# quadram-institute-bioscience/tatajuba

Measured on AMD Instinct MI355X. Metric: reads/s (whole node), 150 bp synthetic FASTQ, homopolymer scan + context histogram, higher is better.
Workload: dtype u8/u64

## Files before the change

tatajuba_amd/csrc/hopo_device.hip:

```cpp

#include <hip/hip_runtime.h>
#include <rccl/rccl.h>
#include <dlfcn.h>
#include <mutex>
#include <string>
#include <new>
#include <stdint.h>
#include <stdio.h>
#include <stdlib.h>
#include <string.h>
#include <stdarg.h>
#include <limits.h>
#include <float.h>
#include <algorithm>
#include <vector>

#include "../../include/tatajuba_amd.h"

typedef unsigned long long u64;
typedef unsigned int u32;


static thread_local char g_err[512] = "";

// ... 1736 lines not shown
#endif
#endif
        const u32 sh = u + u;
        const u32 clo = __builtin_amdgcn_alignbit (w1, w0, sh), chi = __builtin_amdgcn_alignbit (w2, w1, sh);
        const u32 l = clo & vkm;
        const u32 cb = (clo >> vk2) & 3u;
        const u32 r = (u32) ((((u64) chi << 32) | clo) >> (vk2 + len + len)) & vkm;
        u32 rcl = revcomp_v32 (l, M55, vrs), rcr = revcomp_v32 (r, M55, vrs);
        if ((ncand_all >= 0x40000000u)) {
          const u32 nb = bits32 (T.np, (int) u);
          if ((nb << ((v32 - need) & 31u)) != 0u && need <= 32u) {
            rcl = revcomp_v32 (l | (u32) spread_pairs (nb & ((1u << k) - 1u)), M55, vrs);
            rcr = revcomp_v32 (r | (u32) spread_pairs ((nb >> ((u32) k + len)) & ((1u << k) - 1u)), M55, vrs);
          }
        }
        const bool rev = cb >= 2u;
        const u32 c0 = rev ? rcr : l, c1 = rev ? rcl : r;
        const u32 fld24 = __builtin_amdgcn_perm (0u, 0x10140C08u, (cb << 24) | 0x000C0C0Cu);
        const u32 lo = c1 | (len << 24);
        const u32 hi = c0 | fld24;
        STAMP (6);
#if defined(FK_EXP_STOP) && FK_EXP_STOP == 3
        if (ok) asm volatile ("" :: "v"(lo), "v"(hi), "v"(at));
#else
#if defined(FK_EXP_LINEAR)
        {
          const u32 at = lds_collect (araw) + (u32) __builtin_amdgcn_mbcnt_hi ((u32) (okm >> 32), __builtin_amdgcn_mbcnt_lo ((u32) okm, 0u));
          typedef __attribute__((address_space(1))) u64 *gwords_t;
          gwords_t q = (gwords_t) ((u64) (size_t) BK.pool + (((u64) blockIdx.x * 200000u + (at % 200000u)) << 3));
          if (ok) *q = ((u64) hi << 32) | lo;
        }
#elif defined(FK_EXP_SCATTER)
        (void) lds_collect (araw);
        {
          u32 h = __builtin_amdgcn_udot4 (lo, vh0, 0u, false);
          h = __builtin_amdgcn_udot4 (hi & vm27, vh1, h, false);
          const u32 bin = ok ? ((h ^ (h >> 8)) & 255u) : 256u + (u32) lane;
          const u32 r = atomicAdd (&SL.hist[bin], 1u);
          const uint4 e = reinterpret_cast<const uint4 *> (SL.gbase)[bin & 255u];
          asm volatile ("" :: "v"(e.x), "v"(e.y), "v"(e.z), "v"(e.w));
          typedef __attribute__((address_space(1))) u64 *gwords_t;
          gwords_t q = (gwords_t) ((u64) (size_t) BK.pool + ((((u64) (bin & 255u) * 512u + (blockIdx.x & 511u)) * 512u + (r & 511u)) << 3));
          if (ok) *q = ((u64) hi << 32) | lo;
        }
#else
        const u32 at = lds_collect (araw) + (u32) __builtin_amdgcn_mbcnt_hi ((u32) (okm >> 32), __builtin_amdgcn_mbcnt_lo ((u32) okm, 0u));
        if constexpr (LOG) sink.store1ok (ok, at, lo, hi, (u32) lane);
        else sink.store1v (ok ? at : (u32) sink.S + (u32) lane, lo, hi, vh0, vh1, vm27);
#endif
#endif
        STAMP (7);
      }
    }
#if !(defined(FK_EXP_NOBAR) && (FK_EXP_NOBAR & 1))
    lds_barrier ();
#endif
    STAMP (8);
    if (nt >= grp_end) { gpar ^= 1u; grp_end = nt + FK_GROUP; }
    tile = nt;
    it++;
  }
  STAMP_FLUSH;
  flush_slow ();
  sink.finish ();
}

#define PL_BLOCK 512
#ifndef PL_WG_PER_CU
#define PL_WG_PER_CU 2
#endif
template <int W>
__global__ __launch_bounds__ (PL_BLOCK, PL_BLOCK * PL_WG_PER_CU / 256)
void partition_log_kernel (LogSpace LG, Buckets BK, DevCounters *ctr, int k)
{
  static_assert (W == 1 || W == 2, "the log holds one-word and two-word records");
  typedef StageLds<W, 2> Lds;
  __shared__ Lds L;
  constexpr u32 RB = TJ_LOGB / W;
  static_assert (Lds::S == (int) RB && Lds::WS == W, "one pass per log block");
  constexpr u32 RR = RB / PL_BLOCK;
  static_assert (RR % 4 == 0, "bins are kept four to a register");
  const u32 tid = threadIdx.x, lane = tid & 63u;
  const u32 wave = (u32) __builtin_amdgcn_readfirstlane ((int) (tid >> 6));
  if (tid < TJ_P) L.hist[tid] = 0;
  u32 cur_j = TJ_EMPTY, cur_chunk = TJ_NOCHUNK;
  lds_barrier ();
  const u32 n_blocks = min (*LG.next, LG.n_blocks);
#if TJ_STAMPS == 2
  Stamper stamper; stamper.begin ();
#endif
  u32 b = blockIdx.x;
  if (b >= n_blocks) return;
  u64 w[RR][W];
  u32 n = min (LG.count[b], RB), nn = 0;
  auto load_block = [&] (u32 blk, u32 cnt) {
    const u64 *__restrict__ src = LG.log + ((u64) blk << TJ_LOGB_SHIFT);
    const u32 w0 = tid & ~63u;
#pragma unroll
    for (u32 r = 0; r < RR; r++) {
#pragma unroll
      for (int j = 0; j < W; j++) w[r][j] = 0;
      if (w0 + r * PL_BLOCK < cnt) {
        if constexpr (W == 1) w[r][0] = (src + r * PL_BLOCK)[tid];
        else { const ulonglong2 v = reinterpret_cast<const ulonglong2 *> (src + 2u * r * PL_BLOCK)[tid]; w[r][0] = v.x; w[r][1] = v.y; }
      }
    }
  };
  auto bucket_of = [&] (const u64 *rec) -> u32 {
    if constexpr (W == 1) return bucket_of_rec1 ((u32) rec[0], (u32) (rec[0] >> 32));
    else { u64 c0, c1; u32 base, len10, flag; unpack_raw<W> (rec, k, c0, c1, base, len10, flag); return bucket_of_key (c0, c1, base, len10); }
  };
  load_block (b, n);
  while (true) {
    const u32 bn = b + gridDim.x;
    const bool more = bn < n_blocks;
    if (more) nn = min (LG.count[bn], RB);
    PLSTAMP (0);
    u32 tq = tid;
    asm volatile ("" : "+v"(tq));
    u32 pk[RR / 4];
#pragma unroll
    for (u32 r = 0; r < RR / 4; r++) pk[r] = 0;
    if (n) {
#pragma unroll
      for (u32 r = 0; r < RR; r++) {
        const u32 bin = bucket_of (w[r]);
        pk[r >> 2] |= bin << (8u * (r & 3u));
        if (tid + r * PL_BLOCK < n) atomicAdd (&L.hist[bin], 1u);
      }
      PLSTAMP (1);
      lds_barrier ();
      PLSTAMP (2);
      if (wave < TJ_P / 64) {
        const uint4 h4 = *reinterpret_cast<const uint4 *> (&L.hist[4 * lane]);
        const u32 tot = h4.x + h4.y + h4.z + h4.w;
        const u32 e0 = wave_inclusive_scan (tot) - tot;
        if ((lane >> 4) == wave) *reinterpret_cast<uint4 *> (&L.offs[4 * lane]) = make_uint4 (e0, e0 + h4.x, e0 + h4.x + h4.y, e0 + h4.x + h4.y + h4.z);
        const u32 cnt = L.hist[tid], off = L.offs[tid];
        u64 a1 = 0, a2 = 0;
        u32 thr = off + cnt;
        if (cnt) {
          const u32 p0 = atomicAdd (&BK.cursors[tid * TJ_CSTRIDE], cnt);
          const u32 ch = (u32) TJ_CH0 << BK.ch_shift;
          bucket_claim_ahead_range (BK, tid, p0, cnt, ctr);
          const u32 j0 = chunk_of_pos (BK, p0), j1 = chunk_of_pos (BK, p0 + cnt - 1);
          if (j0 != cur_j) { cur_j = j0; cur_chunk = bucket_chunk_id (BK, tid, j0, true, ctr); }
          if (cur_chunk != TJ_NOCHUNK) a1 = (u64) (size_t) (BK.pool + ((u64) cur_chunk * ch + (p0 - j0 * ch)) * W) - (8ull * W) * off;
          if (j1 != j0) {
            thr = off + ((j0 + 1u) * ch - p0);
            cur_j = j0 + 1u; cur_chunk = bucket_chunk_id (BK, tid, j0 + 1u, true, ctr);
            if (cur_chunk != TJ_NOCHUNK) a2 = (u64) (size_t) (BK.pool + ((u64) cur_chunk * ch) * W) - (8ull * W) * thr;
          }
        }
        reinterpret_cast<uint4 *> (L.gbase)[tid] = make_uint4 ((u32) a1, (u32) (a1 >> 32) | (thr << 16), (u32) a2, (u32) (a2 >> 32));
      }
      PLSTAMP (3);
      lds_barrier ();
      PLSTAMP (4);
      if (tid < TJ_P) L.hist[tid] = 0;
#pragma unroll
      for (u32 r = 0; r < RR; r++)
        if (tid + r * PL_BLOCK < n) {
          const u32 bin = (pk[r >> 2] >> (8u * (r & 3u))) & 255u;
          const u32 d = atomicAdd (&L.offs[bin], 1u);
#pragma unroll
          for (int j = 0; j < W; j++) L.rec[d * W + j] = w[r][j];
          L.bin[d] = (unsigned char) bin;
        }
      PLSTAMP (5);
      lds_barrier ();
      PLSTAMP (6);
      for (u32 r0 = 0; r0 < RR; r0 += 4) {
        if (r0 * PL_BLOCK >= n) break;
        u32 cb[4]; uint4 e[4]; u64 cw[4][W];
#pragma unroll
        for (u32 h = 0; h < 4; h++) cb[h] = L.bin[tq + (r0 + h) * PL_BLOCK];
#pragma unroll
        for (u32 h = 0; h < 4; h++) {
          e[h] = reinterpret_cast<const uint4 *> (L.gbase)[cb[h]];
#pragma unroll
          for (int j = 0; j < W; j++) cw[h][j] = L.rec[(tq + (r0 + h) * PL_BLOCK) * W + j];
        }
#pragma unroll
        for (u32 h = 0; h < 4; h++) {
          const u32 i = tq + (r0 + h) * PL_BLOCK;
          const u64 a = (i < (e[h].y >> 16)) ? (((u64) (e[h].y & 0xFFFFu) << 32) | e[h].x) : (((u64) e[h].w << 32) | e[h].z);
          if (i < n && a != 0ull) {
            typedef __attribute__((address_space(1))) u64 *gwords_t;
            gwords_t q = (gwords_t) (a + (u64) (8u * W * i));
#pragma unroll
            for (int j = 0; j < W; j++) q[j] = cw[h][j];
          }
        }
      }
      PLSTAMP (7);
      lds_barrier ();
      PLSTAMP (8);
    }
    if (!more) break;
    load_block (bn, nn);
    n = nn; b = bn;
  }
  PLSTAMP_FLUSH;
}

template <int W>
__global__ void nrun_fixup_bins_kernel (const uint8_t *__restrict__ seq, long n_bytes, int k, int mprime,
                                        Buckets BK, DevCounters *ctr, const FixEntry *fix, u32 fix_cap, int par)
{
  nrun_fixup_entries<W> (seq, n_bytes, k, mprime, BK, ctr, fix, fix_cap, par, blockIdx.x * (u64) blockDim.x + threadIdx.x, (u64) gridDim.x * blockDim.x);
}

template <int W>
__global__ void bin_elems_kernel (const u64 *__restrict__ elems5, long n, int k, Buckets BK, DevCounters *ctr)
{
  for (long i = blockIdx.x * (long) blockDim.x + threadIdx.x; i < n; i += (long) gridDim.x * blockDim.x) {
    const u64 m = elems5[5 * i + 2];
    bucket_insert_slow<W> (elems5[5 * i], elems5[5 * i + 1], (u32) (m & 3ull), (u32) ((m >> TJ_META_LEN_SHIFT) & 0x3FFull),
                           (u32) ((m >> TJ_META_FLAG_SHIFT) & 3ull), k, BK, ctr);
  }
}

template <int W>
__global__ void unpack_buckets_kernel (Buckets BK, int k, u64 *__restrict__ out, u64 cap, u64 *n_out)
{
  const u32 b = blockIdx.x;
  const u32 n = BK.cursors[b * TJ_CSTRIDE];
  for (u32 i = threadIdx.x; i < n; i += blockDim.x) {
    u64 c0, c1; u32 base, len10, flag;
    const u64 at = bucket_slot (BK, b, i, false, nullptr);
    if (at == ~0ull) continue;
    unpack_raw<W> (BK.pool + at * W, k, c0, c1, base, len10, flag);
    if (flag == 3u) continue;
    const u64 o = atomicAdd (n_out, 1ull);
    if (o < cap) { u64 *q = out + 3 * o; q[0] = c0; q[1] = c1; q[2] = make_meta (base, len10, flag); }
  }
}

__global__ void init_table_kernel (u32 *table, u32 maxj, u32 *pool_next)
{
  const u32 b = blockIdx.x * blockDim.x + threadIdx.x;
  if (b < TJ_P) table[(u64) b * maxj] = b;
  if (b == 0) *pool_next = TJ_P;
}

__global__ void clear_buckets_kernel (u32 *cursors, DevCounters *ctr, u32 *table, u32 maxj, int ch_shift, FinCounts *fin, u32 *bins, int nbins,
                                      DevCounters *snap_ctr, u32 *snap_cursors, FinPlan *plan, u32 *__restrict__ fine = nullptr, int fine_bits = 0)
{
  const u32 b = blockIdx.x;
  if (snap_ctr) {
    if (threadIdx.x == 0) {
      snap_cursors[b] = cursors[b * TJ_CSTRIDE];
      if (b == 0) {
        snap_cursors[TJ_P] = cursors[TJ_P * TJ_CSTRIDE];
        if (plan) { plan->n1_exact = (long) fin->n_kept; plan->ovf_exact = fin->overflow; }
      }
    }
    if (b == 0) for (u32 i = threadIdx.x; i < sizeof (DevCounters) / 4; i += blockDim.x) reinterpret_cast<u32 *> (snap_ctr)[i] = reinterpret_cast<const u32 *> (ctr)[i];
    __syncthreads ();
  }
  if (b == 0) for (u32 i = threadIdx.x; i < sizeof (DevCounters) / 4; i += blockDim.x) if (i != offsetof (DevCounters, n_undefined) / 4 && i != offsetof (DevCounters, n_undefined) / 4 + 1) reinterpret_cast<u32 *> (ctr)[i] = 0;
  if (table) {
    u32 used = maxj;
    if (ch_shift >= 0) used = min (maxj, ((cursors[b * TJ_CSTRIDE] / TJ_CH0) >> ch_shift) + 3u);
    for (u32 j = threadIdx.x; j < used; j += blockDim.x) table[(u64) b * maxj + j] = j ? TJ_EMPTY : b;
  }
  if (fine) {
    const int gid = (int) (b * blockDim.x + threadIdx.x), gsz = (int) (gridDim.x * blockDim.x);
    if (plan->ok) {
      const int shift = fine_bits - plan->nbits, run = 1 << shift, nb = plan->nbins;
      for (int i = gid; i < nb; i += gsz) {
        u32 sum = 0;
        if (shift >= 2) {
          uint4 *f4 = reinterpret_cast<uint4 *> (fine) + (size_t) i * (run >> 2);
          for (int j = 0; j < (run >> 2); j++) { const uint4 v = f4[j]; sum += v.x + v.y + v.z + v.w; }
          for (int j = 0; j < (run >> 2); j++) f4[j] = make_uint4 (0, 0, 0, 0);
        }
        else {
          for (int j = 0; j < run; j++) sum += fine[(i << shift) + j];
          for (int j = 0; j < run; j++) fine[(i << shift) + j] = 0;
        }
        bins[i] = sum;
      }
    }
    else for (int i = gid; i < (1 << fine_bits); i += gsz) fine[i] = 0;
  }
  else if (bins) for (int i = (int) (b * blockDim.x + threadIdx.x); i < nbins; i += (int) (gridDim.x * blockDim.x)) bins[i] = 0;
  __syncthreads ();
  if (threadIdx.x == 0) { cursors[b * TJ_CSTRIDE] = 0; if (b == 0) { cursors[TJ_P * TJ_CSTRIDE] = TJ_P; fin->n_kept = 0; fin->overflow = 0; fin->pad = 0; } }
}

__global__ void table_relayout_kernel (const u32 *__restrict__ old, u32 old_maxj, u32 *__restrict__ neu, u32 new_maxj)
{
  const u32 b = blockIdx.x;
  for (u32 j = threadIdx.x; j < old_maxj; j += blockDim.x) neu[(u64) b * new_maxj + j] = old[(u64) b * old_maxj + j];
}


#define AG_BLOCK    1024
#define AG_NCH      512

#define AG1_S        8192
#define AG1_CLOSE_AT 4864
#define AG1_R        4
#define AG1_MARK     (~0ull)

#define BS_MAXBITS   16
__host__ __device__ static inline int cov_table_bits (long n1) { int b = 10; while ((1l << b) < 4 * n1 && b < 31) b++; return b; }
__host__ __device__ static inline int cov_plan_bits (long n1, int k, int *direct)
{
  const int hb = cov_table_bits (n1), kb = 2 * k < 31 ? 2 * k : 31;
  *direct = kb <= hb ? 1 : 0;
  return kb <= hb ? kb : hb;
}
__host__ __device__ static inline int fine_bin_bits (int k) { return BS_MAXBITS < 1 + 4 * k ? BS_MAXBITS : 1 + 4 * k; }
__device__ __forceinline__ u32 bin_of_record (u64 c0, u64 c1, u64 meta, int k, int nbits);
__host__ __device__ static inline int bin_bits_for (long n1, int k)
{
  int nbits = 6;
  while (nbits < BS_MAXBITS && nbits < 1 + 4 * k && (48l << nbits) < n1) nbits++;
  return nbits < 1 + 4 * k ? nbits : 1 + 4 * k;
}
__device__ __forceinline__ void flag_kept_overflow (FinCounts *fin)
{
  u32 old = atomicOr (&fin->overflow, 1u);
  asm volatile ("" :: "v"(old));
}

__device__ __forceinline__ void plan_tail (FinCounts *fin, int k, long cap, FinPlan *plan)
{
  if (!plan) return;
  __syncthreads ();
  if (threadIdx.x == 0) {
    const u32 done = atomicAdd (&fin->pad, 1u);
    if (done == gridDim.x - 1u) {
      const long n1 = (long) __hip_atomic_load (&fin->n_kept, __ATOMIC_RELAXED, __HIP_MEMORY_SCOPE_AGENT);
      const u32 ovf = __hip_atomic_load (&fin->overflow, __ATOMIC_RELAXED, __HIP_MEMORY_SCOPE_AGENT);
      plan->n1 = n1; plan->kept_overflow = ovf;
      plan->nbits = bin_bits_for (n1, k); plan->nbins = 1 << plan->nbits;
      int direct;
      plan->log2t = cov_plan_bits (n1, k, &direct); plan->t = 1l << plan->log2t; plan->cov_direct = (u32) direct;
      plan->ok = (n1 > 0 && n1 <= cap && !ovf) ? 1 : 0;
      fin->pad = 0;
    }
  }
}

#ifndef AG_FROM_END
#define AG_FROM_END 1
#endif
__device__ __forceinline__ u32 batch_start (u32 t, u32 n, u32 batch)
{
#if AG_FROM_END
  const u32 nb = (n + batch - 1u) / batch;
  return t < nb ? (nb - 1u - t) * batch : n;
#else
  return t * batch;
#endif
}

struct Agg1Lds
{
  u64 key[AG1_S];
  u32 cnt[2 * AG1_S];
  u32 chunk[AG_NCH];
  u32 n_claimed, n_ovf, total;
  u32 next_batch;
  u32 wsum[AG_BLOCK / 64];
};

__global__ __launch_bounds__ (AG_BLOCK)
void aggregate1_kernel (Buckets BK, u64 *ovf, int k, int remove_biased, u64 *__restrict__ kept, u64 kept_cap, FinCounts *fin,
                        long plan_cap, FinPlan *plan, u32 *__restrict__ fine, int fine_bits)
{
  __shared__ Agg1Lds L;
  const int tid = threadIdx.x, lane = tid & 63, wave = tid >> 6;
  const u32 bkt = blockIdx.x;
  u32 n = BK.cursors[bkt * TJ_CSTRIDE];
  if (n) for (u32 j = (u32) tid; j <= chunk_of_pos (BK, n - 1u) && j < AG_NCH; j += AG_BLOCK) L.chunk[j] = bucket_chunk_id (BK, bkt, j, false, nullptr);
  auto chunk_id = [&] (u32 j) { return j < AG_NCH ? L.chunk[j] : bucket_chunk_id (BK, bkt, j, false, nullptr); };

  const u64 *src = BK.pool;
  u64 *dst = ovf;
  ASTAMP_DECL;
  while (n > 0) {
    ASTAMP (0);
    for (int i = tid; i < AG1_S; i += AG_BLOCK) { L.key[i] = 0; L.cnt[2 * i] = 0; L.cnt[2 * i + 1] = 0; }
    if (tid == 0) { L.n_claimed = 0; L.n_ovf = 0; L.next_batch = 0; }
    __syncthreads ();

    u64 wn[AG1_R];
    u32 vn = 0;
    auto fetch = [&] (u32 b0) {
      vn = 0;
#pragma unroll
      for (int r = 0; r < AG1_R; r++) wn[r] = 0;
      if (b0 >= n) return;
      const u32 ch = (u32) TJ_CH0 << BK.ch_shift;
      const u32 j0 = chunk_of_pos (BK, b0), bound = (j0 + 1u) * ch;
      if (b0 + 64u * AG1_R <= min (n, bound) && j0 < AG_NCH) {
        const u32 c0s = (u32) __builtin_amdgcn_readfirstlane ((int) L.chunk[j0]);
        if (c0s != TJ_NOCHUNK) {
          const u64 *q = src + ((u64) c0s * ch + (b0 - j0 * ch)) + (u32) lane;
#pragma unroll
          for (int r = 0; r < AG1_R; r++) wn[r] = q[64 * r];
          vn = (1u << AG1_R) - 1u;
          return;
        }
      }
      const u32 c0 = chunk_id (j0), c1 = (bound < n) ? chunk_id (j0 + 1u) : TJ_NOCHUNK;
      const u64 off0 = (u64) c0 * ch - (u64) j0 * ch, off1 = (u64) c1 * ch - (u64) bound;
#pragma unroll
      for (int r = 0; r < AG1_R; r++) {
        const u32 idx = b0 + (u32) r * 64u + (u32) lane;
        const bool hi = idx >= bound;
        if (idx < n && (hi ? c1 : c0) != TJ_NOCHUNK) { vn |= 1u << r; wn[r] = src[(hi ? off1 : off0) + idx]; }
      }
    };
    auto next_batch = [&] () {
      u32 b = 0;
      if (lane == 0) b = atomicAdd (&L.next_batch, 1u);
      return batch_start ((u32) __builtin_amdgcn_readfirstlane ((int) b), n, 64u * AG1_R);
    };
    u32 b_next = next_batch ();
    fetch (b_next);
    ASTAMP (1);
    while (b_next < n) {
      const u32 b0 = b_next;
      (void) b0;
      asm volatile ("s_waitcnt vmcnt(0)" : "+v"(wn[0]), "+v"(wn[1]), "+v"(wn[2]), "+v"(wn[3]) :: "memory");
      static_assert (AG1_R == 4, "asm operand list");
      ASTAMP (2);
      u64 w[AG1_R];
#pragma unroll
      for (int r = 0; r < AG1_R; r++) w[r] = wn[r];
      const u32 valid = vn;
      b_next = next_batch ();
      fetch (b_next);
      ASTAMP (3);
      ASTAMP (4);
#if defined(TJ_EXP_AGG) && TJ_EXP_AGG == 1
      { u64 acc = 0;
#pragma unroll
        for (int r = 0; r < AG1_R; r++) acc ^= w[r];
        if (acc == 0x123456789ull) atomicAdd (&L.n_ovf, 1u);
        continue; }
#endif
      {
        auto home = [] (u64 key) {
          u32 h = (u32) key ^ __builtin_amdgcn_alignbit ((u32) (key >> 32), (u32) (key >> 32), 17);
          h *= 0x9E3779B1u; h ^= h >> 15;
          return h & (AG1_S / 2 - 1);
        };
        u32 todo = 0;
        u32 hp[AG1_R];
        ulonglong2 hk[AG1_R];
#pragma unroll
        for (int r = 0; r < AG1_R; r++) {
          hp[r] = home (w[r] & R1_KEY_MASK);
          hk[r] = *reinterpret_cast<const ulonglong2 *> (&L.key[2 * hp[r]]);
        }
        asm volatile ("" : "+v"(hk[0].x), "+v"(hk[0].y), "+v"(hk[1].x), "+v"(hk[1].y), "+v"(hk[2].x), "+v"(hk[2].y), "+v"(hk[3].x), "+v"(hk[3].y));
#pragma unroll
        for (int r = 0; r < AG1_R; r++) {
          const u64 cur = w[r];
          if (((valid >> r) & 1u) && ((cur >> R1_FLAG_SHIFT) & 3ull) != 3ull) {
            const u64 key = cur & R1_KEY_MASK;
            const bool hx = hk[r].x == key, hy = hk[r].y == key;
            if (hx | hy) atomicAdd (&L.cnt[4 * hp[r] + (hx ? 0u : 2u) + ((u32) (cur >> (R1_FLAG_SHIFT + 1)) & 1u)], 1u);
            else todo |= 1u << r;
          }
        }
        u32 probes = 0;
        u32 r = todo ? (u32) __ffs ((int) todo) - 1u : 0u;
        u64 cur = (r == 0u) ? w[0] : (r == 1u) ? w[1] : (r == 2u) ? w[2] : w[3];
        u32 pair = home (cur & R1_KEY_MASK);
        while (todo) {
          bool adv = false, left = false;
          {
            const u64 key = cur & R1_KEY_MASK;
            const u32 strand = (u32) (cur >> (R1_FLAG_SHIFT + 1)) & 1u;
            const ulonglong2 kk = *reinterpret_cast<const ulonglong2 *> (&L.key[2 * pair]);
            if (kk.x == key || kk.y == key) { atomicAdd (&L.cnt[4 * pair + (kk.x == key ? 0u : 2u) + strand], 1u); adv = true; }
            else {
              const bool e0 = (kk.x == 0ull) | (kk.x == AG1_MARK), e1 = (kk.y == 0ull) | (kk.y == AG1_MARK);
              if (e0 | e1) {
                const u32 slot = 2 * pair + (e0 ? 0u : 1u);
                if ((e0 ? kk.x : kk.y) == AG1_MARK) { left = true; adv = true; }
                else {
                  const bool closed = __hip_atomic_load (&L.n_claimed, __ATOMIC_RELAXED, __HIP_MEMORY_SCOPE_WORKGROUP) > AG1_CLOSE_AT;
                  const u64 old = atomicCAS ((unsigned long long *) &L.key[slot], 0ull, closed ? AG1_MARK : (unsigned long long) key);
                  if (old == 0ull) {
                    if (closed) left = true;
                    else { atomicAdd (&L.n_claimed, 1u); atomicAdd (&L.cnt[2 * slot + strand], 1u); }
                    adv = true;
                  }
                }
              }
              else if (++probes >= AG1_S / 2) { left = true; adv = true; }
              else pair = (pair + 1u) & (AG1_S / 2 - 1);
            }
          }
          if (left) {
            const u32 o = atomicAdd (&L.n_ovf, 1u);
            const u32 j = chunk_of_pos (BK, o), oc = chunk_id (j);
            if (oc != TJ_NOCHUNK) dst[(((u64) oc * TJ_CH0) << BK.ch_shift) + (o - ((j * TJ_CH0) << BK.ch_shift))] = cur;
          }
          if (adv) {
            todo &= todo - 1u; probes = 0;
            if (todo) {
              r = (u32) __ffs ((int) todo) - 1u;
              cur = (r == 1u) ? w[1] : (r == 2u) ? w[2] : w[3];
              pair = home (cur & R1_KEY_MASK);
            }
          }
        }
      }
      ASTAMP (5);
    }
    __syncthreads ();
    ASTAMP (6);

    u32 mine = 0;
    u64 metas[AG1_S / AG_BLOCK];
#pragma unroll
    for (int r = 0; r < AG1_S / AG_BLOCK; r++) {
      const int slot = tid + r * AG_BLOCK;
      metas[r] = 0;
      if (L.key[slot] && L.key[slot] != AG1_MARK) {
        const u32 cf = L.cnt[2 * slot], cr = L.cnt[2 * slot + 1];
        const u64 flag = (cf ? 1ull : 0ull) | (cr ? 2ull : 0ull);
        const u64 cnt = ((u64) cf + (u64) cr) & 0xFFFFFull;
        const int scnt = (cnt & 0x80000ull) ? (int) cnt - 0x100000 : (int) cnt;
        if (remove_biased ? (flag == 3ull) : (scnt > 1)) {
          const u64 key = L.key[slot];
          const u64 len10 = ((key >> 24) & 0xFFull) | (((key >> 56) & 3ull) << 8);
          metas[r] = ((key >> 58) & 1ull) | (len10 << TJ_META_LEN_SHIFT) | (cnt << TJ_META_COUNT_SHIFT) |
                     (0xffeull << TJ_META_MISM_SHIFT) | (flag << TJ_META_FLAG_SHIFT);
          mine++;
        }
      }
    }
    const u32 x = wave_inclusive_scan (mine);
    if (lane == 63) L.wsum[wave] = x;
    __syncthreads ();
    u32 wbase = 0, total = 0;
    for (int wv = 0; wv < AG_BLOCK / 64; wv++) { const u32 sm = L.wsum[wv]; if (wv < wave) wbase += sm; total += sm; }
    if (tid == 0) L.total = total ? atomicAdd (&fin->n_kept, total) : 0u;
    __syncthreads ();
    u64 at = (u64) L.total + wbase + x - mine;
#pragma unroll
    for (int r = 0; r < AG1_S / AG_BLOCK; r++)
      if (metas[r]) {
        const u64 key = L.key[tid + r * AG_BLOCK];
        if (at < kept_cap) {
          u64 *q = kept + 3 * at; q[0] = (key >> 32) & 0xFFFFFFull; q[1] = key & 0xFFFFFFull; q[2] = metas[r];
          if (fine) atomicAdd (&fine[bin_of_record ((key >> 32) & 0xFFFFFFull, key & 0xFFFFFFull, metas[r], k, fine_bits)], 1u);
        }
        else flag_kept_overflow (fin);
        at++;
      }
    __threadfence_block ();
    __syncthreads ();
    n = L.n_ovf;
    { const u64 *t = src; src = dst; dst = (u64 *) t; }
    __syncthreads ();
    ASTAMP (7);
  }
  ASTAMP_FLUSH;
  plan_tail (fin, k, plan_cap, plan);
}

#define AG2_S        6144
#define AG2_PAIRS    (AG2_S / 2)
#ifndef AG2_CLOSE_AT
#define AG2_CLOSE_AT 2560
#endif
#define AG2_R        4
#define AG2_VALID    (1ull << 63)
#define AG2_PENDING  (1ull << 63)
#define AG2_MARK     (1ull << 63)

struct Agg2Lds
{
  ulonglong2 kk[AG2_S];
  u32 cnt[2 * AG2_S];
  u32 chunk[AG_NCH];
  u32 n_claimed, n_ovf, total;
  u32 next_batch;
  u32 wsum[AG_BLOCK / 64];
};

__global__ __launch_bounds__ (AG_BLOCK)
void aggregate2_kernel (Buckets BK, u64 *ovf, int k, int remove_biased, u64 *__restrict__ kept, u64 kept_cap, FinCounts *fin,
                        long plan_cap, FinPlan *plan, u32 *__restrict__ fine, int fine_bits)
{
  __shared__ Agg2Lds L;
  const int tid = threadIdx.x, lane = tid & 63, wave = tid >> 6;
  const u32 bkt = blockIdx.x;
  u32 n = BK.cursors[bkt * TJ_CSTRIDE];
  const u64 m56 = (1ull << 56) - 1ull, fmask = ~(3ull << 61);
  if (n) for (u32 j = (u32) tid; j <= chunk_of_pos (BK, n - 1u) && j < AG_NCH; j += AG_BLOCK) L.chunk[j] = bucket_chunk_id (BK, bkt, j, false, nullptr);
  auto chunk_id = [&] (u32 j) { return j < AG_NCH ? L.chunk[j] : bucket_chunk_id (BK, bkt, j, false, nullptr); };
  const u64 *src = BK.pool;
  u64 *dst = ovf;

  while (n > 0) {
    for (int i = tid; i < AG2_S; i += AG_BLOCK) { L.kk[i] = make_ulonglong2 (0ull, 0ull); L.cnt[2 * i] = 0; L.cnt[2 * i + 1] = 0; }
    if (tid == 0) { L.n_claimed = 0; L.n_ovf = 0; L.next_batch = 0; }
    __syncthreads ();

    u64 wn[2 * AG2_R];
    u32 vn = 0;
    auto fetch = [&] (u32 b0) {
      vn = 0;
#pragma unroll
      for (int r = 0; r < 2 * AG2_R; r++) wn[r] = 0;
      if (b0 >= n) return;
      const u32 ch = (u32) TJ_CH0 << BK.ch_shift;
      const u32 j0 = chunk_of_pos (BK, b0), bound = (j0 + 1u) * ch;
      const u32 c0 = chunk_id (j0), c1 = (bound < n) ? chunk_id (j0 + 1u) : TJ_NOCHUNK;
      const u64 off0 = (u64) c0 * ch - (u64) j0 * ch, off1 = (u64) c1 * ch - (u64) bound;
#pragma unroll
      for (int r = 0; r < AG2_R; r++) {
        const u32 idx = b0 + (u32) r * 64u + (u32) lane;
        const bool hi = idx >= bound;
        if (idx < n && (hi ? c1 : c0) != TJ_NOCHUNK) {
          const ulonglong2 v = *reinterpret_cast<const ulonglong2 *> (src + 2 * ((hi ? off1 : off0) + idx));
          vn |= 1u << r; wn[2 * r] = v.x; wn[2 * r + 1] = v.y;
        }
      }
    };
    auto next_batch = [&] () {
      u32 b = 0;
      if (lane == 0) b = atomicAdd (&L.next_batch, 1u);
      return batch_start ((u32) __builtin_amdgcn_readfirstlane ((int) b), n, 64u * AG2_R);
    };
    u32 b_next = next_batch ();
    fetch (b_next);
    while (b_next < n) {
      asm volatile ("s_waitcnt vmcnt(0)" : "+v"(wn[0]), "+v"(wn[1]), "+v"(wn[2]), "+v"(wn[3]), "+v"(wn[4]), "+v"(wn[5]), "+v"(wn[6]), "+v"(wn[7]) :: "memory");
      static_assert (AG2_R == 4, "asm operand list");
      u64 w[2 * AG2_R];
#pragma unroll
      for (int r = 0; r < 2 * AG2_R; r++) w[r] = wn[r];
      const u32 valid = vn;
      b_next = next_batch ();
      fetch (b_next);
      {
        auto home = [] (u64 a, u64 b) {
          const u64 key1 = b & ~(3ull << 61);
          u32 h = (u32) a ^ __builtin_amdgcn_alignbit ((u32) (a >> 32), (u32) (a >> 32), 19) ^
                  __builtin_amdgcn_alignbit ((u32) key1, (u32) key1, 11) ^ __builtin_amdgcn_alignbit ((u32) (key1 >> 32), (u32) (key1 >> 32), 25);
          h *= 0x9E3779B1u; h ^= h >> 15;
          return __umulhi (h, (u32) AG2_PAIRS);
        };
        auto load_pair = [&] (u32 pair, ulonglong2 &s0, ulonglong2 &s1) {
          s0.x = __hip_atomic_load ((unsigned long long *) &L.kk[2 * pair].x, __ATOMIC_RELAXED, __HIP_MEMORY_SCOPE_WORKGROUP);
          s0.y = __hip_atomic_load ((unsigned long long *) &L.kk[2 * pair].y, __ATOMIC_RELAXED, __HIP_MEMORY_SCOPE_WORKGROUP);
          s1.x = __hip_atomic_load ((unsigned long long *) &L.kk[2 * pair + 1].x, __ATOMIC_RELAXED, __HIP_MEMORY_SCOPE_WORKGROUP);
          s1.y = __hip_atomic_load ((unsigned long long *) &L.kk[2 * pair + 1].y, __ATOMIC_RELAXED, __HIP_MEMORY_SCOPE_WORKGROUP);
        };
        u32 todo = 0, look = 0, cur[AG2_R];
#pragma unroll
        for (int q = 0; q < AG2_R; q++) {
          cur[q] = 0;
          if (((valid >> q) & 1u) && ((w[2 * q + 1] >> 61) & 3ull) != 3ull) { look |= 1u << q; cur[q] = home (w[2 * q], w[2 * q + 1]); }
        }
#pragma unroll
        for (int pass = 0; pass < 3; pass++) {
          if (pass && !look) break;
#pragma unroll
          for (int q = 0; q < AG2_R; q++)
            if ((look >> q) & 1u) {
              const u64 a0 = w[2 * q], a1 = w[2 * q + 1];
              ulonglong2 s0, s1;
              load_pair (cur[q], s0, s1);
              const u64 want = (a1 & fmask) | AG2_VALID;
              const bool m0 = (s0.x == a0) & (s0.y == want), m1 = (s1.x == a0) & (s1.y == want);
              if (m0 | m1) { atomicAdd (&L.cnt[2 * (2 * cur[q] + (m0 ? 0u : 1u)) + ((u32) (a1 >> 62) & 1u)], 1u); look &= ~(1u << q); }
              else {
                const u64 mine = a0 | AG2_PENDING;
                const bool o0 = (s0.x != 0ull) & (s0.x != AG2_MARK) & (s0.x != mine) & ((s0.x & AG2_PENDING) == 0ull) & ((s0.x != a0) | ((s0.y & AG2_VALID) != 0ull));
                const bool o1 = (s1.x != 0ull) & (s1.x != AG2_MARK) & (s1.x != mine) & ((s1.x & AG2_PENDING) == 0ull) & ((s1.x != a0) | ((s1.y & AG2_VALID) != 0ull));
                if (o0 & o1) cur[q] = (cur[q] + 1u == (u32) AG2_PAIRS) ? 0u : cur[q] + 1u;
                else { look &= ~(1u << q); todo |= 1u << q; }
              }
            }
        }
        todo |= look;
        u32 probes = 0;
        u32 r = todo ? (u32) __ffs ((int) todo) - 1u : 0u;
        u64 w0 = (r == 0u) ? w[0] : (r == 1u) ? w[2] : (r == 2u) ? w[4] : w[6];
        u64 w1 = (r == 0u) ? w[1] : (r == 1u) ? w[3] : (r == 2u) ? w[5] : w[7];
        u32 pair = (r == 0u) ? cur[0] : (r == 1u) ? cur[1] : (r == 2u) ? cur[2] : cur[3];
        while (todo) {
          bool adv = false, left = false;
          {
            const u64 key1 = w1 & fmask, want = key1 | AG2_VALID;
            const u32 strand = (u32) (w1 >> 62) & 1u;
            ulonglong2 s0, s1;
            load_pair (pair, s0, s1);
            const bool m0 = (s0.x == w0) & (s0.y == want), m1 = (s1.x == w0) & (s1.y == want);
            const bool again = (s0.x == (w0 | AG2_PENDING)) | (s1.x == (w0 | AG2_PENDING)) |
                               ((s0.x == w0) & !(s0.y & AG2_VALID)) | ((s1.x == w0) & !(s1.y & AG2_VALID));
            if (m0 | m1) { atomicAdd (&L.cnt[2 * (2 * pair + (m0 ? 0u : 1u)) + strand], 1u); adv = true; }
            else if (!again) {
              const bool e0 = (s0.x == 0ull) | (s0.x == AG2_MARK), e1 = (s1.x == 0ull) | (s1.x == AG2_MARK);
              if (e0 | e1) {
                const u32 slot = 2 * pair + (e0 ? 0u : 1u);
                if ((e0 ? s0.x : s1.x) == AG2_MARK) { left = true; adv = true; }
                else {
                  const bool closed = __hip_atomic_load (&L.n_claimed, __ATOMIC_RELAXED, __HIP_MEMORY_SCOPE_WORKGROUP) > AG2_CLOSE_AT;
                  const u64 old = atomicCAS ((unsigned long long *) &L.kk[slot].x, 0ull, closed ? AG2_MARK : (unsigned long long) (w0 | AG2_PENDING));
                  if (old == 0ull) {
                    if (closed) left = true;
                    else {
                      __hip_atomic_store ((unsigned long long *) &L.kk[slot].y, (unsigned long long) want, __ATOMIC_RELAXED, __HIP_MEMORY_SCOPE_WORKGROUP);
                      atomicAdd (&L.n_claimed, 1u);
                      __hip_atomic_store ((unsigned long long *) &L.kk[slot].x, (unsigned long long) w0, __ATOMIC_RELEASE, __HIP_MEMORY_SCOPE_WORKGROUP);
                      atomicAdd (&L.cnt[2 * slot + strand], 1u);
                    }
                    adv = true;
                  }
                }
              }
              else if (++probes >= AG2_PAIRS) { left = true; adv = true; }
              else pair = (pair + 1u == (u32) AG2_PAIRS) ? 0u : pair + 1u;
            }
          }
          if (left) {
            const u32 o = atomicAdd (&L.n_ovf, 1u);
            const u32 j = chunk_of_pos (BK, o), oc = chunk_id (j);
            if (oc != TJ_NOCHUNK) {
              const u64 at = (((u64) oc * TJ_CH0) << BK.ch_shift) + (o - ((j * TJ_CH0) << BK.ch_shift));
              dst[2 * at] = w0; dst[2 * at + 1] = w1;
            }
          }
          if (adv) {
            todo &= todo - 1u; probes = 0;
            if (todo) {
              r = (u32) __ffs ((int) todo) - 1u;
              w0 = (r == 1u) ? w[2] : (r == 2u) ? w[4] : w[6];
              w1 = (r == 1u) ? w[3] : (r == 2u) ? w[5] : w[7];
              pair = (r == 1u) ? cur[1] : (r == 2u) ? cur[2] : cur[3];
            }
          }
        }
      }
    }
    __syncthreads ();

    u32 mine = 0;
    u64 metas[AG2_S / AG_BLOCK];
#pragma unroll
    for (int r = 0; r < AG2_S / AG_BLOCK; r++) {
      const int slot = tid + r * AG_BLOCK;
      metas[r] = 0;
      if (L.kk[slot].x && L.kk[slot].x != AG2_MARK) {
        const u32 cf = L.cnt[2 * slot], cr = L.cnt[2 * slot + 1];
        const u64 flag = (cf ? 1ull : 0ull) | (cr ? 2ull : 0ull);
        const u64 cnt = ((u64) cf + (u64) cr) & 0xFFFFFull;
        const int scnt = (cnt & 0x80000ull) ? (int) cnt - 0x100000 : (int) cnt;
        if (remove_biased ? (flag == 3ull) : (scnt > 1)) {
          const u64 a = L.kk[slot].x, b = L.kk[slot].y;
          const u64 len10 = ((a >> 2) & 31ull) | (((b >> 56) & 31ull) << 5);
          metas[r] = ((a >> 1) & 1ull) | (len10 << TJ_META_LEN_SHIFT) | (cnt << TJ_META_COUNT_SHIFT) |
                     (0xffeull << TJ_META_MISM_SHIFT) | (flag << TJ_META_FLAG_SHIFT);
          mine++;
        }
      }
    }
    const u32 x = wave_inclusive_scan (mine);
    if (lane == 63) L.wsum[wave] = x;
    __syncthreads ();
    u32 wbase = 0, total = 0;
    for (int wv = 0; wv < AG_BLOCK / 64; wv++) { const u32 sm = L.wsum[wv]; if (wv < wave) wbase += sm; total += sm; }
    if (tid == 0) L.total = total ? atomicAdd (&fin->n_kept, total) : 0u;
    __syncthreads ();
    u64 at = (u64) L.total + wbase + x - mine;
#pragma unroll
    for (int r = 0; r < AG2_S / AG_BLOCK; r++)
      if (metas[r]) {
        const int slot = tid + r * AG_BLOCK;
        if (at < kept_cap) {
          u64 *q = kept + 3 * at; q[0] = (L.kk[slot].x >> 7) & m56; q[1] = L.kk[slot].y & m56; q[2] = metas[r];
          if (fine) atomicAdd (&fine[bin_of_record ((L.kk[slot].x >> 7) & m56, L.kk[slot].y & m56, metas[r], k, fine_bits)], 1u);
        }
        else flag_kept_overflow (fin);
        at++;
      }
    __threadfence_block ();
    __syncthreads ();
    n = L.n_ovf;
    { const u64 *t = src; src = dst; dst = (u64 *) t; }
    __syncthreads ();
  }
  plan_tail (fin, k, plan_cap, plan);
}

#define AG4_S        4096
#define AG4_CLOSE_AT 2560
#define AG4_R        2
#define AG4_PENDING  (1ull << 63)
#define AG4_MARK     (1ull << 63)

struct Agg4Lds
{
  u64 cw[AG4_S], c0[AG4_S], c1[AG4_S];
  u32 cnt[2 * AG4_S];
  u32 chunk[AG_NCH];
  u32 n_claimed, n_ovf, total;
  u32 next_batch;
  u32 wsum[AG_BLOCK / 64];
};

// ... 3356 lines not shown
```

Baseline: 11.44 billion.

## Double per-lane aggregation batch and hash to single slot instead of bucket pair

Raises the number of records each lane fetches and aggregates per batch from four to eight, so more global loads are in flight per wait. The LDS hash now homes each key to a single slot, so the fast-path lookup reads one 64-bit key instead of a 128-bit pair. The slow-path probe still scans slot pairs, starting at the homed slot's partner ordering. A branchless select replaces the ternary chain for picking the pending record. This costs more registers per lane, which may lower occupancy, and single-slot homing may push more keys onto the slower probe path.

```diff
diff --git a/tatajuba_amd/csrc/hopo_device.hip b/tatajuba_amd/csrc/hopo_device.hip
--- a/tatajuba_amd/csrc/hopo_device.hip
+++ b/tatajuba_amd/csrc/hopo_device.hip
@@ -2062,7 +2062,7 @@
 
 #define AG1_S        8192
 #define AG1_CLOSE_AT 4864
-#define AG1_R        4
+#define AG1_R        8
 #define AG1_MARK     (~0ull)
 
 #define BS_MAXBITS   16
@@ -2188,8 +2188,8 @@
     while (b_next < n) {
       const u32 b0 = b_next;
       (void) b0;
-      asm volatile ("s_waitcnt vmcnt(0)" : "+v"(wn[0]), "+v"(wn[1]), "+v"(wn[2]), "+v"(wn[3]) :: "memory");
-      static_assert (AG1_R == 4, "asm operand list");
+      asm volatile ("s_waitcnt vmcnt(0)" : "+v"(wn[0]), "+v"(wn[1]), "+v"(wn[2]), "+v"(wn[3]), "+v"(wn[4]), "+v"(wn[5]), "+v"(wn[6]), "+v"(wn[7]) :: "memory");
+      static_assert (AG1_R == 8, "asm operand lists");
       ASTAMP (2);
       u64 w[AG1_R];
 #pragma unroll
@@ -2210,43 +2210,48 @@
         auto home = [] (u64 key) {
           u32 h = (u32) key ^ __builtin_amdgcn_alignbit ((u32) (key >> 32), (u32) (key >> 32), 17);
           h *= 0x9E3779B1u; h ^= h >> 15;
-          return h & (AG1_S / 2 - 1);
+          return h & (AG1_S - 1);
         };
         u32 todo = 0;
-        u32 hp[AG1_R];
-        ulonglong2 hk[AG1_R];
+        u32 hs[AG1_R];
+        u64 hk[AG1_R];
 #pragma unroll
         for (int r = 0; r < AG1_R; r++) {
-          hp[r] = home (w[r] & R1_KEY_MASK);
-          hk[r] = *reinterpret_cast<const ulonglong2 *> (&L.key[2 * hp[r]]);
+          hs[r] = home (w[r] & R1_KEY_MASK);
+          hk[r] = L.key[hs[r]];
         }
-        asm volatile ("" : "+v"(hk[0].x), "+v"(hk[0].y), "+v"(hk[1].x), "+v"(hk[1].y), "+v"(hk[2].x), "+v"(hk[2].y), "+v"(hk[3].x), "+v"(hk[3].y));
+        asm volatile ("" : "+v"(hk[0]), "+v"(hk[1]), "+v"(hk[2]), "+v"(hk[3]), "+v"(hk[4]), "+v"(hk[5]), "+v"(hk[6]), "+v"(hk[7]));
 #pragma unroll
         for (int r = 0; r < AG1_R; r++) {
           const u64 cur = w[r];
           if (((valid >> r) & 1u) && ((cur >> R1_FLAG_SHIFT) & 3ull) != 3ull) {
-            const u64 key = cur & R1_KEY_MASK;
-            const bool hx = hk[r].x == key, hy = hk[r].y == key;
-            if (hx | hy) atomicAdd (&L.cnt[4 * hp[r] + (hx ? 0u : 2u) + ((u32) (cur >> (R1_FLAG_SHIFT + 1)) & 1u)], 1u);
+            if (hk[r] == (cur & R1_KEY_MASK)) atomicAdd (&L.cnt[2 * hs[r] + ((u32) (cur >> (R1_FLAG_SHIFT + 1)) & 1u)], 1u);
             else todo |= 1u << r;
           }
         }
+        auto pick = [&] (u32 r) { u64 c = 0;
+#pragma unroll
+                                  for (int i = 0; i < AG1_R; i++) c |= w[i] & (0ull - (u64) (r == (u32) i));
+                                  return c; };
         u32 probes = 0;
         u32 r = todo ? (u32) __ffs ((int) todo) - 1u : 0u;
-        u64 cur = (r == 0u) ? w[0] : (r == 1u) ? w[1] : (r == 2u) ? w[2] : w[3];
-        u32 pair = home (cur & R1_KEY_MASK);
+        u64 cur = pick (r);
+        u32 pair = home (cur & R1_KEY_MASK), lo = pair & 1u;
+        pair >>= 1;
         while (todo) {
           bool adv = false, left = false;
           {
             const u64 key = cur & R1_KEY_MASK;
             const u32 strand = (u32) (cur >> (R1_FLAG_SHIFT + 1)) & 1u;
             const ulonglong2 kk = *reinterpret_cast<const ulonglong2 *> (&L.key[2 * pair]);
-            if (kk.x == key || kk.y == key) { atomicAdd (&L.cnt[4 * pair + (kk.x == key ? 0u : 2u) + strand], 1u); adv = true; }
+            const u64 ka = lo ? kk.y : kk.x, kb = lo ? kk.x : kk.y;
+            const u32 sa = 2 * pair + lo, sb = sa ^ 1u;
+            if (ka == key || kb == key) { atomicAdd (&L.cnt[2 * (ka == key ? sa : sb) + strand], 1u); adv = true; }
             else {
-              const bool e0 = (kk.x == 0ull) | (kk.x == AG1_MARK), e1 = (kk.y == 0ull) | (kk.y == AG1_MARK);
-              if (e0 | e1) {
-                const u32 slot = 2 * pair + (e0 ? 0u : 1u);
-                if ((e0 ? kk.x : kk.y) == AG1_MARK) { left = true; adv = true; }
+              const bool ea = (ka == 0ull) | (ka == AG1_MARK), eb = (kb == 0ull) | (kb == AG1_MARK);
+              if (ea | eb) {
+                const u32 slot = ea ? sa : sb;
+                if ((ea ? ka : kb) == AG1_MARK) { left = true; adv = true; }
                 else {
                   const bool closed = __hip_atomic_load (&L.n_claimed, __ATOMIC_RELAXED, __HIP_MEMORY_SCOPE_WORKGROUP) > AG1_CLOSE_AT;
                   const u64 old = atomicCAS ((unsigned long long *) &L.key[slot], 0ull, closed ? AG1_MARK : (unsigned long long) key);
@@ -2258,7 +2263,7 @@
                 }
               }
               else if (++probes >= AG1_S / 2) { left = true; adv = true; }
-              else pair = (pair + 1u) & (AG1_S / 2 - 1);
+              else { pair = (pair + 1u) & (AG1_S / 2 - 1); lo = 0u; }
             }
           }
           if (left) {
@@ -2270,8 +2275,8 @@
             todo &= todo - 1u; probes = 0;
             if (todo) {
               r = (u32) __ffs ((int) todo) - 1u;
-              cur = (r == 1u) ? w[1] : (r == 2u) ? w[2] : w[3];
-              pair = home (cur & R1_KEY_MASK);
+              cur = pick (r);
+              pair = home (cur & R1_KEY_MASK); lo = pair & 1u; pair >>= 1;
             }
           }
         }
```

Result: no change. 11.40 billion (median of 2 runs) (-0.4%).
